# adamfilli/happy-simulator

Hardware: AMD Instinct MI355X
Metric: committed events/sec (whole node), 65 536-server M/M/1 grid (higher is better)
Workload: dtype int64+f64

## Files before the change

### happy_simulator_amd/csrc/hs_device.hpp

```cpp
#pragma once

#include <hip/hip_runtime.h>
#include <stdint.h>

namespace hs {

constexpr int64_t kInfNs = INT64_MAX;
constexpr double kMaxReachNs = 9.0e18;
constexpr double kLongestExpDraw = 36.8;
inline bool reach_fits_int64(int64_t horizon_ns, double step_s) { return (double)horizon_ns + step_s * 1e9 < kMaxReachNs; }

enum StreamKind : uint32_t { kStreamArrival = 0, kStreamService = 1, kStreamLink = 2, kStreamRoute = 3, kStreamKey = 4, kStreamLoss = 5 };

struct U4 { uint32_t x, y, z, w; };

__device__ __forceinline__ U4 philox4x32_10(uint32_t c0, uint32_t c1, uint32_t c2, uint32_t c3, uint32_t k0,
                                            uint32_t k1) {
#pragma unroll
    for (int r = 0; r < 10; ++r) {
        const uint64_t p0 = (uint64_t)0xD2511F53u * (uint64_t)c0, p1 = (uint64_t)0xCD9E8D57u * (uint64_t)c2;
        const uint32_t hi0 = (uint32_t)(p0 >> 32), lo0 = (uint32_t)p0;
        const uint32_t hi1 = (uint32_t)(p1 >> 32), lo1 = (uint32_t)p1;
        c0 = hi1 ^ c1 ^ k0;
        c1 = lo1;
// ... 53 lines not shown
    return __fma_rn(r1, 1e-9, q1);
}
__device__ __forceinline__ double ns_from_seconds_d(double x) { return __builtin_trunc(__dmul_rn(x, 1e9)); }
__device__ __forceinline__ double seconds_from_ns_d(double ns) {
    const double q0 = __dmul_rn(ns, 1e-9);
    const double r0 = __fma_rn(-1e9, q0, ns);
    const double q1 = __fma_rn(r0, 1e-9, q0);
    const double r1 = __fma_rn(-1e9, q1, ns);
    return __fma_rn(r1, 1e-9, q1);
}
__device__ __forceinline__ int64_t i64_from_whole_d(double d) {
    return (int64_t)((uint64_t)__double_as_longlong(__dadd_rn(d, 4503599627370496.0)) & 0xFFFFFFFFFFFFFull);
}
__device__ __forceinline__ double seconds_from_ns_ieee(int64_t ns) { return __ddiv_rn(__ll2double_rn(ns), 1e9); }

struct ConstDiv {
    double b, y;
    bool fast;
    __device__ __forceinline__ void init(double divisor) {
        b = divisor;
        y = __ddiv_rn(1.0, divisor);
        const uint64_t bits = (uint64_t)__double_as_longlong(divisor);
        const uint32_t ex = (uint32_t)(bits >> 52) & 0x7ffu;
        const bool all_ones = (bits & 0x000fffffffffffffull) == 0x000fffffffffffffull;
        fast = !all_ones && ex > 1023u - 200u && ex < 1023u + 200u && (bits >> 63) == 0;
    }
    __device__ __forceinline__ double div(double a) const {
        if (!fast) return __ddiv_rn(a, b);
        const double q0 = __dmul_rn(a, y);
        const double r0 = __fma_rn(-b, q0, a);
        const double q1 = __fma_rn(r0, y, q0);
        const double r1 = __fma_rn(-b, q1, a);
        return __fma_rn(r1, y, q1);
    }
};

struct Stream {
    uint32_t key0, key1, sid0, sid1;
    uint64_t k;
    uint32_t c2, c3;

    __device__ __forceinline__ void init(uint64_t seed, uint64_t sid, uint64_t k0) {
        key0 = (uint32_t)seed; key1 = (uint32_t)(seed >> 32);
// ... 85 lines not shown
```

### happy_simulator_amd/csrc/hs_engine.hip

```cpp
#include <hip/hip_runtime.h>

#include <cmath>
#include <cstdio>
#include <cstdlib>
#include <cstring>
#include <algorithm>
#include <new>
#include <string>
#include <vector>
#include <map>
#include <mutex>
#include <utility>

#define HS_KERNELS_MAIN
#include "hs_kernels.hpp"
#include "hs_tables_api.hpp"
#include "hs_host.hpp"
#include "hs_plan.hpp"

struct hs_engine {
    bool pending_async = false;

    hs_config cfg{};
    int C = 1;
// ... 1634 lines not shown
    if (!h || !o) return fail(h, HS_E_INVALID, "hs_engine_get_lp_stats: null argument");
    if (!h->have_stations) return fail(h, HS_E_STATE, "stations not set");
    if (h) { const int rcf = results_final(h); if (rcf) return rcf; }
    HS_HIP(h, hipSetDevice(h->cfg.device));
    HS_HIP(h, hipStreamSynchronize(h->stream));
    const size_t n = (size_t)h->cfg.n_lp;
#define DL(dst, src, T) if (o->dst) HS_HIP(h, hipMemcpy(o->dst, h->X.src, n * sizeof(T), hipMemcpyDeviceToHost))
    DL(generated, generated, int64_t); DL(accepted, accepted, int64_t); DL(dropped, dropped, int64_t);
    DL(completed, completed, int64_t); DL(rejected, rejected, int64_t); DL(total_service_s, total_service, double);
    DL(sink_received, received, int64_t); DL(queue_depth, buf, int64_t); DL(active, active, int32_t);
    DL(events, events, int64_t); DL(final_time_ns, last_time, int64_t);
#undef DL
    return HS_OK;
}

int64_t hs_engine_read_sink(hs_engine *h, int32_t lp, int64_t *t_ns, int64_t *created_ns, int64_t cap) {
    if (!h || !h->have_stations) return fail(h, HS_E_STATE, "stations not set");
    if (lp < 0 || lp >= h->cfg.n_lp) return fail(h, HS_E_INVALID, "LP index %d out of range", lp);
    if (h) { const int rcf = results_final(h); if (rcf) return rcf; }
    if (hipSetDevice(h->cfg.device) != hipSuccess || hipStreamSynchronize(h->stream) != hipSuccess)
        return fail(h, HS_E_HIP, "device synchronisation failed");
    int64_t cnt = 0;
    if (hipMemcpy(&cnt, h->X.received + lp, 8, hipMemcpyDeviceToHost) != hipSuccess) return fail(h, HS_E_HIP, "memcpy");
    if (cnt > h->L.cap) cnt = h->L.cap;
    if (cnt > cap) cnt = cap;
    if (cnt > 0) {
        int64_t *tmp = nullptr;
        if (hipMalloc(&tmp, (size_t)cnt * 8) != hipSuccess) return fail(h, HS_E_HIP, "hipMalloc of the read-back staging buffer failed");
        const int64_t *cols[2] = {h->L.sink_t, h->L.sink_created};
        int64_t *dsts[2] = {t_ns, created_ns};
        for (int c = 0; c < 2; ++c) {
            if (!dsts[c]) continue;
            hipLaunchKernelGGL(hs_gather_one, dim3((unsigned)((cnt + 255) / 256)), dim3(256), 0, h->stream, cols[c], tmp,
                               h->cfg.n_lp, lp, cnt, h->L.lp_major ? h->L.cap : (int64_t)0);
            if (hipStreamSynchronize(h->stream) != hipSuccess ||
                hipMemcpy(dsts[c], tmp, (size_t)cnt * 8, hipMemcpyDeviceToHost) != hipSuccess) {
                hipFree(tmp);
                return fail(h, HS_E_HIP, "sink read-back failed");
            }
        }
        hipFree(tmp);
    }
    return cnt;
}

int64_t hs_engine_read_sinks(hs_engine *h, int64_t *counts, int64_t *t_ns, int64_t *created_ns, int64_t cap_total) {
    if (!h || !h->have_stations) return fail(h, HS_E_STATE, "stations not set");
    if (!counts) return fail(h, HS_E_INVALID, "counts is required");
    if (h) { const int rcf = results_final(h); if (rcf) return rcf; }
    if (hipSetDevice(h->cfg.device) != hipSuccess || hipStreamSynchronize(h->stream) != hipSuccess)
        return fail(h, HS_E_HIP, "device synchronisation failed");
    const size_t n = (size_t)h->cfg.n_lp;
    if (hipMemcpy(counts, h->X.received, n * 8, hipMemcpyDeviceToHost) != hipSuccess) return fail(h, HS_E_HIP, "memcpy");
    const int64_t cap = h->L.cap;
    std::vector<int64_t> off(n);
    int64_t total = 0, maxc = 0;
// ... 11 lines not shown
        return fail(h, HS_E_HIP, "hipMalloc of the read-back staging buffers failed");
    }
    bool ok = hipMemcpy(d_off, off.data(), n * 8, hipMemcpyHostToDevice) == hipSuccess;
    const int64_t *cols[2] = {h->L.sink_t, h->L.sink_created};
    int64_t *dsts[2] = {t_ns, created_ns};
    for (int c = 0; c < 2 && ok; ++c) {
        if (!dsts[c]) continue;
        const dim3 grid((unsigned)((n + 63) / 64), (unsigned)((maxc + 63) / 64));
        hipLaunchKernelGGL(hs_gather_logs, grid, dim3(256), 0, h->stream, cols[c], h->X.received, d_off, d_out, (int)n, cap, (int)h->L.lp_major);
        ok = hipStreamSynchronize(h->stream) == hipSuccess &&
             hipMemcpy(dsts[c], d_out, (size_t)total * 8, hipMemcpyDeviceToHost) == hipSuccess;
    }
    hipFree(d_off);
    hipFree(d_out);
    if (!ok) return fail(h, HS_E_HIP, "sink read-back failed");
    return total;
}

int64_t hs_engine_read_probe(hs_engine *h, int32_t lp, int64_t *t_ns, int64_t *values, int64_t cap) {
    return hs_engine_read_probe_slot(h, lp, 0, t_ns, values, cap);
}

int hs_engine_read_source_generated(hs_engine *h, int32_t slot, int64_t *out) {
    if (!h || !h->have_stations || !out) return fail(h, HS_E_STATE, "stations not set");
    if (slot < 0 || slot > kMaxXSrc) return fail(h, HS_E_INVALID, "source slot %d out of range", slot);
    const size_t n = (size_t)h->cfg.n_lp;
    if (h) { const int rcf = results_final(h); if (rcf) return rcf; }
    HS_HIP(h, hipSetDevice(h->cfg.device));
    HS_HIP(h, hipStreamSynchronize(h->stream));
    if (slot == 0) { HS_HIP(h, hipMemcpy(out, h->X.generated, n * 8, hipMemcpyDeviceToHost)); return HS_OK; }
// ... 167 lines not shown
```

### happy_simulator_amd/csrc/hs_kernels.hpp

```cpp
#pragma once

#include <hip/hip_runtime.h>

#include "../../include/hs_engine.h"
#include "hs_netstation.hpp"
#ifdef HS_KERNELS_MAIN
#include "hs_exact.hpp"
#endif

using namespace hs;

namespace {

template <typename T>
__device__ __forceinline__ T wave_sum(T v) {
#pragma unroll
    for (int o = 32; o > 0; o >>= 1) v += __shfl_xor(v, o, 64);
    return v;
}

__device__ __forceinline__ long long shfl_xor_ll(long long v, int o) {
    int lo = (int)(unsigned)(v & 0xffffffffll), hi = (int)(v >> 32);
    lo = __shfl_xor(lo, o, 64);
    hi = __shfl_xor(hi, o, 64);
// ... 430 lines not shown
    const int lp = blockIdx.x * kBlock + tid;
    const bool live = lp < n && !producer;
    if (threadIdx.x < 12) red[threadIdx.x] = 0;
    if (threadIdx.x == 0) { red_time = INT64_MIN; red_flags[0] = 0; red_flags[1] = 0; }
    if constexpr (PC) {
        if (!producer) { pc_prod[tid] = 0; pc_cons[tid] = 0; if ((tid & 63) == 0) pc_done[tid >> 6] = 0; }
    }
    const long long cur = tot->cur_time;
    __syncthreads();

    Station<C, PF, UNI> S;
    Candidate mine;
    mine = cand_none(lp);
    if constexpr (PC) {
        if (producer) {
            const int w = tid >> 6;
            bool wants_a = false, wants_s = false;
            uint64_t gen_a = 0, gen_s = 0;
            uint32_t prod_a = 0, prod_s = 0;
            int slot_a = 0, slot_s = 0;
            if (lp < n) {
                S.tid = tid;
                S.rate = P.src_rate[lp];
                S.svc_lambda = __ddiv_rn(1.0, P.svc_mean[lp]);
                S.prof_kind = kProfConstant;
                S.init_streams(P.seed[lp], P.stream_base[lp], X.arr_k[lp], X.svc_k[lp], ring_a, ring_s);
                wants_a = P.src_kind[lp] == 1 && X.A[lp] != kInfNs;
                wants_s = P.svc_kind[lp] == 0;
                gen_a = S.arr_k; gen_s = S.svc_k;
            }
            for (;;) {
                if (__hip_atomic_load(&pc_done[w], __ATOMIC_RELAXED, __HIP_MEMORY_SCOPE_WORKGROUP)) break;
                const uint32_t c = __hip_atomic_load(&pc_cons[tid], __ATOMIC_RELAXED, __HIP_MEMORY_SCOPE_WORKGROUP);
                const uint32_t out_a = (prod_a - (c & 0xffffu)) & 0xffffu, out_s = (prod_s - (c >> 16)) & 0xffffu;
                const bool do_a = wants_a && out_a + (uint32_t)kRefill <= (uint32_t)kRing;
                const bool do_s = wants_s && out_s + (uint32_t)kRefill <= (uint32_t)kRing;
                if (!__any(do_a || do_s)) { __builtin_amdgcn_s_sleep(HS_PC_SLEEP_P); continue; }
                if (__any(do_a)) {
                    if (do_a) {
                        const uint64_t b0 = gen_a >> 1;
                        const bool odd = (gen_a & 1) != 0;
#pragma unroll
                        for (int i = 0; i < kRefill / 2; ++i) {
                            const uint64_t b = b0 + (uint64_t)i;
                            const U4 o = philox4x32_10((uint32_t)b, (uint32_t)(b >> 32), S.asid0, S.asid1, S.key0, S.key1);
                            const double v0 = S.arr_value(res53(o.x, o.y)), v1 = S.arr_value(res53(o.z, o.w));
                            if (!(i == 0 && odd)) { ring_a[slot_a][tid] = v0; slot_a = slot_a + 1 == kRing ? 0 : slot_a + 1; ++prod_a; ++gen_a; }
                            ring_a[slot_a][tid] = v1; slot_a = slot_a + 1 == kRing ? 0 : slot_a + 1; ++prod_a; ++gen_a;
                        }
                    }
                }
                if (__any(do_s)) {
                    if (do_s) {
                        const uint64_t b0 = gen_s >> 1;
                        const bool odd = (gen_s & 1) != 0;
#pragma unroll
                        for (int i = 0; i < kRefill / 2; ++i) {
                            const uint64_t b = b0 + (uint64_t)i;
                            const U4 o = philox4x32_10((uint32_t)b, (uint32_t)(b >> 32), S.ssid0, S.ssid1, S.key0, S.key1);
                            const double v0 = S.svc_value(res53(o.x, o.y)), v1 = S.svc_value(res53(o.z, o.w));
                            if (!(i == 0 && odd)) { ring_s[slot_s][tid] = v0; slot_s = slot_s + 1 == kRing ? 0 : slot_s + 1; ++prod_s; ++gen_s; }
                            ring_s[slot_s][tid] = v1; slot_s = slot_s + 1 == kRing ? 0 : slot_s + 1; ++prod_s; ++gen_s;
                        }
                    }
                }
                __hip_atomic_store(&pc_prod[tid], (prod_a & 0xffffu) | (prod_s << 16), __ATOMIC_RELEASE, __HIP_MEMORY_SCOPE_WORKGROUP);
            }
        }
    }
    if (live) {
        load_station<C, PF, UNI>(S, P, X, L, lp, n, qmem, ring_a, ring_s, tid);
        S.force_general = (flags & 1) != 0 || (PF && S.trk && (S.n_up > 0 || S.egress == kEgressServer));
    }
    const bool ended = (mode == HS_MODE_REPLICAS) ? (live && S.last_time > end_ns) : (cur > end_ns);
    bool other_pass = false;
    if constexpr (PF) {
        const int pass1 = (flags >> 28) & 7;
        if (pass1 != 0 && live && P.tabs != nullptr && P.tabs->tandem != nullptr) other_pass = P.tabs->tandem[(size_t)kMaxUp * n + lp] != pass1 - 1;
// ... 6 lines not shown
        S.last_time = S.grp_time;
        pre_group = true;
    }
    if constexpr (C == 1) {
        bool bail_reload = false;
        if (!producer) {
            const bool elig = live && !frozen && !pre_group && S.qn == 0 && S.req_eligible();
            typename Station<C, PF, UNI>::ReqCursor rc;
            rc.bail = false; rc.done = true;
            if (elig) S.req_begin(rc, end_ns);
#ifdef HS_CYCLES
            unsigned long long cyc_top = 0, cyc_step = 0, n_it = 0;
#endif
            uint32_t seen = 0;
            const uint64_t ak0 = S.arr_k, sk0 = S.svc_k;
            for (;;) {
                const bool act = elig && !rc.bail && !rc.done;
                if (!__any(act)) break;
#ifdef HS_CYCLES
                const unsigned long long c0 = __builtin_readcyclecounter();
#endif
                if constexpr (PC) {
                    const bool need_a = act && S.src_kind == 1 && S.A != kInfNs, need_s = act && S.svc_kind == 0;
                    const uint32_t ca = (uint32_t)(S.arr_k - ak0) & 0xffffu, cs = (uint32_t)(S.svc_k - sk0) & 0xffffu;
                    unsigned spins = 0;
                    while (__any((need_a && (seen & 0xffffu) == ca) || (need_s && (seen >> 16) == cs))) {
                        seen = __hip_atomic_load(&pc_prod[tid], __ATOMIC_ACQUIRE, __HIP_MEMORY_SCOPE_WORKGROUP);
                        if (__any((need_a && (seen & 0xffffu) == ca) || (need_s && (seen >> 16) == cs))) __builtin_amdgcn_s_sleep(HS_PC_SLEEP_C);
                        if (++spins > (1u << 22)) {
                            if (elig) { S.qoverflow = 1; rc.done = true; }
                            break;
                        }
                    }
                    if (spins > (1u << 22)) continue;
                } else {
                    S.top_up(act);
                }
#ifdef HS_CYCLES
                const unsigned long long c1 = __builtin_readcyclecounter();
#endif
                S.req_step(rc, act);
                if constexpr (PC) {
                    __hip_atomic_store(&pc_cons[tid], ((uint32_t)(S.arr_k - ak0) & 0xffffu) | ((uint32_t)(S.svc_k - sk0) << 16),
                                       __ATOMIC_RELAXED, __HIP_MEMORY_SCOPE_WORKGROUP);
                    seen = __hip_atomic_load(&pc_prod[tid], __ATOMIC_ACQUIRE, __HIP_MEMORY_SCOPE_WORKGROUP);
                }
#ifdef HS_CYCLES
                const unsigned long long c2 = __builtin_readcyclecounter();
                cyc_top += c1 - c0; cyc_step += c2 - c1; ++n_it;
#endif
            }
#ifdef HS_CYCLES
            if ((tid & 63) == 0) {
                atomicAdd(&tot->dbg[0], cyc_top); atomicAdd(&tot->dbg[1], cyc_step);
                atomicAdd(&tot->dbg[2], n_it); atomicAdd(&tot->dbg[3], 1ull);
            }
#endif
            if constexpr (PC) {
                if ((tid & 63) == 0) __hip_atomic_store(&pc_done[tid >> 6], 1, __ATOMIC_RELAXED, __HIP_MEMORY_SCOPE_WORKGROUP);
            }
            if (elig && !rc.bail) { S.req_finish(rc); event_order = false; }
            bail_reload = elig && rc.bail;
        }
        if constexpr (PC) __syncthreads();
        if (!producer) {
            if constexpr (PC) {
                S.ra.head = 0; S.ra.n = 0; S.rs.head = 0; S.rs.n = 0;
            }
            if (bail_reload) {
                load_station<C, PF, UNI>(S, P, X, L, lp, n, qmem, ring_a, ring_s, tid);
                S.force_general = (flags & 1) != 0 || (PF && S.trk && (S.n_up > 0 || S.egress == kEgressServer));
            }
        }
        if (!producer) {
            for (;;) {
// ... 1290 lines not shown
```

### happy_simulator_amd/csrc/hs_kernels_wave.hpp

```cpp
#pragma once

constexpr int kWaveR = 128;
constexpr int kWaveRowPad = kWaveR + 2;

namespace {

__device__ __forceinline__ double wave_shr1(double v) {
    const long long b = __double_as_longlong(v);
    int lo = (int)(unsigned)(b & 0xffffffffll), hi = (int)(b >> 32);
    lo = __builtin_amdgcn_update_dpp(lo, lo, 0x138, 0xf, 0xf, false);
    hi = __builtin_amdgcn_update_dpp(hi, hi, 0x138, 0xf, 0xf, false);
    return __longlong_as_double(((long long)hi << 32) | (unsigned)lo);
}
__device__ __forceinline__ MaxPlus mp_after(const MaxPlus &f2, const MaxPlus &f1) {
    return MaxPlus{__builtin_fmax(f2.p, f1.p + f2.q), f1.q + f2.q};
}
template <int CTRL, int RM>
__device__ __forceinline__ MaxPlus mp_scan_step(const MaxPlus &F) {
    return mp_after(F, MaxPlus{dpp_orneg<CTRL, RM>(F.p), dpp_or0<CTRL, RM>(F.q)});
}
__device__ __forceinline__ double rl64(double v, int l) {
    const long long b = __double_as_longlong(v);
    const unsigned lo = (unsigned)__builtin_amdgcn_readlane((int)(unsigned)(b & 0xffffffffll), l);
    const unsigned hi = (unsigned)__builtin_amdgcn_readlane((int)(b >> 32), l);
// ... 52 lines not shown
    for (int k = 0; k < 8; ++k) ev[k] = 0;
    uint32_t c_tick = 0, c_start = 0, c_dep = 0, seq = I.seq, seqA = I.seqA, seqD = I.seqD;
    int64_t acc2 = accepted, st2 = started, A_next_i = A, crtA2 = crtA0, rcA = I.rcA, rcD = I.rcD;
    int32_t dpA = I.dpA, dpD = I.dpD;
    if (count) {
        c_tick = O.n_tick; c_start = O.n_start; c_dep = O.n_dep;
        const uint32_t c_notify = O.n_notify, c_poll = O.n_poll;
        ev[0] = c_tick; ev[1] = c_tick; ev[2] = c_notify; ev[3] = c_poll + c_dep; ev[4] = c_start; ev[5] = c_start; ev[6] = c_dep; ev[7] = c_dep;
        acc2 = accepted + c_tick; st2 = started + c_start;
        A_next_i = A != kInfNs ? to_i64(A_next) : A;
        crtA2 = c_tick ? to_i64(a_last) : crtA0;
        if ((c_tick | c_start) != 0u) {
            const bool d_first = pend && pendS < crtA2;
            seqA = seq + (d_first ? 1u : 0u); seqD = seq + (d_first ? 0u : 1u); seq += 2u;
        }
        if (c_tick) { dpA = 1; rcA = acc2 >= 2 ? (c_tick >= 2 ? to_i64(a_last2) : L.adm[(size_t)(acc2 - 2) * n + lp]) : crtA0; }
        if (pend && pend_new) {
            const int64_t m = st2 - 1;
            if (pendS == to_i64(pendA_d)) {
                dpD = 6;
                rcD = m >= 1 ? (pend_i >= 1 ? to_i64(pendAp_d) : (m - 1 < L.cap ? L.adm[(size_t)(m - 1) * n + lp] : 0)) : crtA0;
            } else {
                dpD = 4; rcD = to_i64(pendSp_d);
            }
        }
        const int64_t Dn = pend ? pendD : kInfNs;
        const int64_t tmin = A_next_i < Dn ? A_next_i : Dn;
        if (tmin != kInfNs) {
            const bool tick_first = A_next_i < Dn || (A_next_i == Dn && (int32_t)(seqA - seqD) < 0);
            mine.t = tmin; mine.valid = 1;
            if (tick_first) { mine.t_created = crtA2; mine.depth = dpA; mine.rcrt = rcA; mine.pad = 2; }
            else { mine.t_created = pend ? pendS : 0; mine.depth = dpD; mine.rcrt = rcD; mine.pad = 0; }
            mine.rank = cand_rank(P, lp, n, mine.pad);
        }
    }
    if constexpr (FRESH) {
// ... 440 lines not shown
```

### happy_simulator_amd/csrc/hs_kernels_wide.hpp

```cpp
#pragma once

namespace {

struct MaxPlus { double p, q; };
__device__ __forceinline__ MaxPlus mp_compose(const MaxPlus &f2, const MaxPlus &f1) {
    const double a = f1.p + f2.q;
    return MaxPlus{f2.p > a ? f2.p : a, f1.q + f2.q};
}
__device__ __forceinline__ double shfl_f64(double v, int src) {
    const long long b = __double_as_longlong(v);
    int lo = (int)(unsigned)(b & 0xffffffffll), hi = (int)(b >> 32);
    lo = __shfl(lo, src, 64);
    hi = __shfl(hi, src, 64);
    return __longlong_as_double(((long long)hi << 32) | (unsigned)lo);
}
__device__ __forceinline__ int64_t shfl_i64(int64_t v, int src) {
    int lo = (int)(unsigned)(v & 0xffffffffll), hi = (int)(v >> 32);
    lo = __shfl(lo, src, 64);
    hi = __shfl(hi, src, 64);
    return ((int64_t)hi << 32) | (unsigned)lo;
}

}

// ... 306 lines not shown
        X.total_service[lp] = total_service;
        const int64_t A_next_i = run && A != kInfNs ? (int64_t)A_next : A;
        X.A[lp] = A_next_i; X.arr_time[lp] = A_next_i; X.arr_k[lp] = ak0 + (uint64_t)n_arr_total; X.svc_k[lp] = sk0 + (uint64_t)c_start;
        const int64_t crtA2 = c_tick ? (int64_t)a_last : crtA0;
        X.crtA[lp] = crtA2;
        uint32_t seq = X.seq[lp];
        uint32_t seqA = X.seqA[lp], seqD = X.seqD[lp];
        if ((c_tick | c_start) != 0u) {
            const bool d_first = pend && pendS < crtA2;
            seqA = seq + (d_first ? 1u : 0u); seqD = seq + (d_first ? 0u : 1u); seq += 2u;
            X.seqA[lp] = seqA; X.seqD[lp] = seqD; X.seq[lp] = seq;
        }
        X.last_time[lp] = lt;
        int32_t dpA = X.dpA[lp], dpD = X.dpD[lp];
        int64_t rcA = X.rcA[lp], rcD = X.rcD[lp];
        if (c_tick) { dpA = 1; rcA = acc2 >= 2 ? (c_tick >= 2 ? (int64_t)a_last2 : L.adm[(size_t)(acc2 - 2) * n + lp]) : crtA0; X.dpA[lp] = (uint8_t)dpA; X.rcA[lp] = rcA; }
        if (pend && pn) {
            const int64_t m = st2 - 1;
            const int64_t a_m = m < L.cap ? L.adm[(size_t)m * n + lp] : 0;
            if (pendS == a_m) { dpD = 6; rcD = m >= 1 ? L.adm[(size_t)(m - 1) * n + lp] : crtA0; }
            else {
                Stream st;
                st.init(((uint64_t)key1 << 32) | key0, ((uint64_t)ssid1 << 32) | ssid0, (uint64_t)(m - 1));
                const double s_prev = seconds_from_ns(ns_from_seconds(div_lambda.div(exp1_from_uniform(st.next_uniform()))));
                dpD = 4; rcD = pendS - ns_from_seconds(s_prev);
            }
            X.dpD[lp] = (uint8_t)dpD; X.rcD[lp] = rcD;
        }
        uint32_t tot_ev = 0;
#pragma unroll
        for (int k = 0; k < 8; ++k) { X.ev_kind[(size_t)k * n + lp] += ev[k]; tot_ev += ev[k]; }
        X.events[lp] += tot_ev;
        const int64_t Dn = pend ? pendD : kInfNs;
        const int64_t tmin = A_next_i < Dn ? A_next_i : Dn;
        if (tmin != kInfNs) {
// ... 148 lines not shown
```

### happy_simulator_amd/csrc/hs_plan.hpp

```cpp
#pragma once

#include <algorithm>
#include <cmath>
#include <cstdarg>
#include <cstdio>
#include <string>
#include <utility>
#include <vector>

#include "../../include/hs_engine.h"
#include "hs_netstation.hpp"
#include "hs_exact.hpp"
#include "hs_tables.hpp"

namespace hs {

inline int fail(std::string &err, int code, const char *fmt, ...) {
    char buf[512];
    va_list ap;
    va_start(ap, fmt);
    vsnprintf(buf, sizeof buf, fmt, ap);
    va_end(ap);
    err = buf;
    return code;
// ... 80 lines not shown
            if (st->src_more_stop_after_ns) p.xsrc_stop[o] = st->src_more_stop_after_ns[o];
            ++p.n_xsrc_total;
        }
    p.any_xsrc = p.n_xsrc_total > 0;
    p.uni_stations = true;
    for (int i = 0; i < n; ++i) {
        if (c.src_kind[i] != HS_SRC_POISSON || c.conc[i] != 1 || c.svc_kind[i] != HS_LAT_EXPONENTIAL || c.qcap[i] >= 0 ||
            c.src_stop[i] >= 0) { p.uni_stations = false; break; }
    }
    p.uni_grid = p.uni_stations;
    for (int i = 0; i < n && p.uni_grid; ++i) if (c.egress[i] != HS_EGRESS_SINK) p.uni_grid = false;
    p.f64_times = cfg.start_ns >= 0 && cfg.horizon_ns < (1ll << 51);
    for (int i = 0; i < n && p.f64_times; ++i)
        if (!(c.svc_mean[i] < 1e4) || !(c.src_rate[i] > 1e-3)) p.f64_times = false;
    if (!p.f64_times) p.uni_grid = false;
    if (p.any_xsrc) p.any_profile = true;
    for (int i = 0; i < n; ++i) {
        const int sk = c.src_kind[i];
        if (sk < 0 || sk > 2) return fail(err, HS_E_INVALID, "LP %d: unknown source kind %d", i, sk);
        if (sk != HS_SRC_NONE) {
            if (!st->src_rate) return fail(err, HS_E_INVALID, "src_rate is required when sources exist");
            const double r = st->src_rate[i];
            if (!(r > 0.0) || !std::isfinite(r))
                return fail(err, HS_E_INVALID, "LP %d: source rate must be > 0 (got %g)", i, r);
            if (r > 1e8) return fail(err, HS_E_UNSUPPORTED, "LP %d: source rate %g above 1e8/s is not supported", i, r);
            const double m = (r + p.xsum[(size_t)i]) * p.horizon_s;
            if (m > p.max_mean_records) p.max_mean_records = m;
            p.reach_s = std::max(p.reach_s, kLongestExpDraw / r);
        }
        const int cc = c.conc[i];
// ... 633 lines not shown
```

### happy_simulator_amd/csrc/hs_station.hpp

```cpp
#pragma once

#include "hs_device.hpp"
#include "hs_tables.hpp"

namespace hs {

enum : uint32_t { Q_PSAMPLE = 0, Q_ENQ = 1, Q_NOTIFY = 2, Q_POLL = 3, Q_DELIVER = 4, Q_TICK = 5, Q_CONT = 6, Q_SINK = 7 };
constexpr int kMaxProbes = 4;
constexpr int kRootProbe = 100;
constexpr int kMaxXSrc = 3;
constexpr int kRootXSrc = 120;
__device__ __forceinline__ uint64_t xsrc_stream_id(uint64_t lp_stream_base, int j) {
    return stream_id((1ull << 40) | (lp_stream_base << 2) | (uint64_t)j, kStreamArrival);
}
constexpr int kRootSched = 98;
constexpr int kRootInj = 200;
constexpr int kMaxUp = 4;
constexpr int kMaxInjRun = 32;
constexpr uint32_t kEgressServer = 4;

constexpr int kBlock = 256;
constexpr int kQCap = 48;
#ifndef HS_KRING
#define HS_KRING 24
// ... 99 lines not shown
    int64_t *XA, *crtX, *x_arr, *x_n;
    uint32_t *seqX;
    uint64_t *x_k;
};

struct RecordLogs {
    int64_t *adm;
    int64_t *sink_t;
    int64_t *sink_created;
    int64_t *sink_created_own;
    int64_t cap;
    int64_t *probe_t, *probe_v;
    int64_t pcap;
    int32_t lp_major;
};
__device__ __forceinline__ size_t log_at(const RecordLogs &L, int64_t k, int lp, int n) {
    return L.lp_major ? (size_t)lp * (size_t)L.cap + (size_t)k : (size_t)k * (size_t)n + (size_t)lp;
}

struct Totals {
    unsigned long long ev[15];
    unsigned long long completed;
    unsigned long long received;
    long long final_time;
    long long cur_time;
    int overflow;
    int qoverflow;
    unsigned int done;
    int undecided;
    unsigned long long dbg[4];
// ... 133 lines not shown
    static __device__ __forceinline__ int32_t rk_place(int64_t w) { return (int32_t)(w & 0xff) - (int32_t)((w >> 40) & 0xff); }
    __device__ __forceinline__ int32_t dp_next(int steps) const { return cd + steps > 255 ? 255 : cd + steps; }

    __device__ __forceinline__ void init_streams(uint64_t seed, uint64_t base, uint64_t ak, uint64_t sk,
                                                 double (*ring_a)[kBlock], double (*ring_s)[kBlock]) {
        key0 = (uint32_t)seed; key1 = (uint32_t)(seed >> 32);
        const uint64_t sa = stream_id(base, kStreamArrival), ss = stream_id(base, kStreamService);
        asid0 = (uint32_t)sa; asid1 = (uint32_t)(sa >> 32);
        ssid0 = (uint32_t)ss; ssid1 = (uint32_t)(ss >> 32);
        arr_k = ak; svc_k = sk;
        ra.reset(ring_a, tid); rs.reset(ring_s, tid);
        div_rate.init(rate);
        div_lambda.init(svc_lambda);
        inc_const = __ddiv_rn(1.0, rate);
    }
    __device__ __forceinline__ double arr_value(double u) const { return div_rate.div(exp1_from_uniform(u)); }
    __device__ __forceinline__ double svc_value(double u) const {
        const double sample = div_lambda.div(exp1_from_uniform(u));
        if constexpr (UNI) return seconds_from_ns_d(ns_from_seconds_d(sample));
        return seconds_from_ns(ns_from_seconds(sample));
    }
    template <int BLOCKS>
    __device__ __forceinline__ void refill_arr() {
        const uint64_t kg = arr_k + (uint64_t)ra.n;
        const uint64_t b0 = kg >> 1;
        const bool odd = (kg & 1) != 0;
#pragma unroll
        for (int i = 0; i < BLOCKS; ++i) {
            const uint64_t b = b0 + (uint64_t)i;
            const U4 o = philox4x32_10((uint32_t)b, (uint32_t)(b >> 32), asid0, asid1, key0, key1);
            const double v0 = arr_value(res53(o.x, o.y)), v1 = arr_value(res53(o.z, o.w));
            if (!(i == 0 && odd)) ra.push(v0);
            ra.push(v1);
// ... 75 lines not shown
        accepted++;
        buf++;
        return was_empty;
    }
    __device__ __forceinline__ bool do_notify() { ev[2]++; return active < conc; }
    __device__ __forceinline__ bool do_poll() {
        ev[3]++;
        if (buf == 0) return false;
        buf--;
        return true;
    }
    __device__ __forceinline__ uint32_t do_deliver_work(int64_t t) {
        ev[4]++;
        ev[5]++;
        const int64_t k = started++;
        if (active >= conc) { rejected++; return 0; }
        active++;
        double s; int64_t dur;
        sample_service(s, dur);
        int j = 0;
#pragma unroll
        for (int i = C - 1; i >= 0; --i) if (D[i] == kInfNs) j = i;
        const int64_t d = t + dur;
        uint32_t same = 0;
#pragma unroll
        for (int i = 0; i < C; ++i) if (i == j) {
            svc_s[i] = s;
            if (C > 1) crt[i] = (k < cap) ? adm[k * ls] : 0;
            if (d == t) { D[i] = kInfNs - 1; same = (uint32_t)i + 1; }
            else { D[i] = d; seqD[i] = seq++; crtD[i] = t; dpD[i] = dp_next(2); rcD[i] = cr; if constexpr (PF) { wkD[i] = wk + 1; lsrcD[i] = lsrc; } }
        }
// ... 497 lines not shown
        last_time = fast ? t : last_time;
        if (slow) run_group(t);
    }

    struct ReqCursor {
        int64_t T;
        int64_t Sprev, Dprev;
        int64_t nb;
        int64_t pendD, pendS;
        double pend_s;
        int64_t lt;
        uint32_t n_tick, n_notify, n_poll, n_start, n_dep;
        bool pend, blocked, bail, done;
        int64_t crtA0;
        double arr_d;
        int64_t pTa, pTd;
        uint32_t ma, md, mf;
        int64_t p_prev;
    };
    __device__ __forceinline__ bool req_eligible() const {
        return C == 1 && !force_general && qn == 0 && conc == 1 && qcap < 0 && stop_ns < 0 && svc_kind != 2 &&
               !(PF && (prof_kind != kProfConstant || n_probes > 1 || has_sched() || has_xsrc() || n_up > 0)) &&
               (egress == 0 || egress == 1) && !(buf > 0 && active == 0) && active <= 1;
    }
    __device__ __forceinline__ int64_t req_probe_time(uint32_t m) {
        return tick_lookup(tab_p[0], tab_cap, p_arr[0] + (int64_t)m, overflow);
    }
    __device__ __forceinline__ void req_probe_begin(ReqCursor &c) {
        c.ma = c.md = c.mf = 0;
        c.pTa = c.pTd = n_probes == 1 ? PA[0] : kInfNs;
// ... 38 lines not shown
                    case kProbeDropped: v = dropped; break;
                    case kProbeCompleted: v = cn; break;
                    case kProbeReceived: v = egress == 1 ? received + c_rel : received; break;
                    case kProbeGenerated: v = generated + g_rel; break;
                    default: break;
                }
                probe_t[o] = req_probe_time(c.mf);
                probe_v[o] = v;
            }
            ++c.mf;
        }
    }
    __device__ __forceinline__ void req_count_departure(ReqCursor &c, bool p, int64_t d, double s) {
        total_service = p ? __dadd_rn(total_service, s) : total_service;
        if (p && HSG(egress == 1, true)) {
            const int64_t w = sink_w + (int64_t)c.n_dep;
            if (w < cap) sink_t[w * ls] = d; else overflow = 1;
        }
        c.n_dep += p ? 1u : 0u;
        c.lt = (p && d > c.lt) ? d : c.lt;
    }
    __device__ __forceinline__ void req_begin(ReqCursor &c, int64_t T) {
        c.T = T; c.nb = buf; c.lt = last_time; c.crtA0 = crtA; c.arr_d = (double)arr_time;
        c.n_tick = c.n_notify = c.n_poll = c.n_start = c.n_dep = 0;
        c.blocked = c.bail = c.done = false;
        const bool busy = active > 0;
        c.Sprev = busy ? crtD[0] : INT64_MIN;
        c.Dprev = busy ? D[0] : INT64_MIN;
        const bool dep0 = busy && D[0] <= T;
        req_count_departure(c, dep0, D[0], svc_s[0]);
        c.pend = busy && !dep0;
        c.pendD = D[0]; c.pendS = crtD[0]; c.pend_s = svc_s[0];
        if constexpr (PF) {
            req_probe_begin(c);
            if (n_probes == 1 && busy) {
                req_probe_departures(c, true, D[0], 0);
                c.bail = c.bail || c.pTd == D[0];
            }
        }
    }
    __device__ __forceinline__ void req_step(ReqCursor &c, bool act) {
        const int64_t T = c.T;
        const bool bk = c.nb > 0 && !c.blocked;
        const bool arr = !bk && A <= T;
        const bool fin = !bk && !arr;
        const double inc = HSG(src_kind == 1, true) ? ra.peek() : inc_const;
        const double a2d = UNI ? ns_from_seconds_d(__dadd_rn(seconds_from_ns_d(c.arr_d), inc)) : 0.0;
        const int64_t a2 = UNI ? i64_from_whole_d(a2d) : ns_from_seconds(__dadd_rn(seconds_from_ns(arr_time), inc));
        const bool tie_a = arr && (A == c.Sprev || A == c.Dprev || a2 <= A);
        const bool notify = arr && c.Sprev < A;
        const bool idle = arr && c.Dprev < A;
        const int64_t Sk = bk ? c.Dprev : (A > c.Dprev ? A : c.Dprev);
        const bool st = (bk || arr) && Sk <= T;
        const double s_new = HSG(svc_kind == 0, true) ? rs.peek() : svc_const_s;
        const int64_t dur = UNI ? i64_from_whole_d(ns_from_seconds_d(s_new)) : (HSG(svc_kind == 0, true) ? ns_from_seconds(s_new) : svc_const_ns);
        const int64_t Dk = Sk + dur;
        const bool dp = st && Dk <= T;
        bool tie_p = false;
        if constexpr (PF) {
            const bool pon = act && n_probes == 1;
            if (__any(pon)) {
                req_probe_arrivals(c, pon && (arr || fin), arr ? A : T + 1, (int64_t)c.n_tick);
                req_probe_departures(c, pon && (st || fin), st ? Dk : T + 1, (int64_t)c.n_dep);
                tie_p = pon && ((arr && c.pTa == A) || (st && c.pTd == Dk));
            }
        }
        const bool bail = act && (tie_a || tie_p || (st && dur == 0));
        const bool go = act && !bail && !fin;
        c.bail = c.bail || bail;
        c.done = c.done || (act && fin);
        const bool arr_g = go && arr, st_g = go && st, dp_g = go && dp;
        if (arr_g) {
            const int64_t w = accepted + (int64_t)c.n_tick;
            if (w < cap) adm[w * ls] = A; else overflow = 1;
        }
        c.n_tick += arr_g ? 1u : 0u;
        c.n_notify += (go && notify) ? 1u : 0u;
        c.n_poll += (go && idle) ? 1u : 0u;
        c.lt = (arr_g && A > c.lt) ? A : c.lt;
        crtA = arr_g ? A : crtA;
        arr_time = arr_g ? a2 : arr_time;
        if constexpr (UNI) c.arr_d = arr_g ? a2d : c.arr_d;
        const bool pop_a = arr_g && HSG(src_kind == 1, true);
        ra.advance_if(pop_a);
        arr_k += pop_a ? 1u : 0u;
        c.n_start += st_g ? 1u : 0u;
        c.lt = (st_g && Sk > c.lt) ? Sk : c.lt;
        const bool pop_s = st_g && HSG(svc_kind == 0, true);
        rs.advance_if(pop_s);
        svc_k += pop_s ? 1u : 0u;
// ... 46 lines not shown
                if (n_probes == 1) {
                    const int64_t tP = crtP[0];
                    const bool p_before_a = tP < crtA, p_before_d = !c.pend || tP < c.pendS;
                    sP = (p_before_a ? 0u : 1u) + ((c.pend && !p_before_d) ? 1u : 0u);
                    sA += p_before_a ? 1u : 0u;
                    sD += p_before_d ? 1u : 0u;
                    seqP[0] = seq + sP;
                }
            }
            seqA = seq + sA;
            seqD[0] = seq + sD;
            seq += 3u;
        }
        if (c.n_tick != 0u) {
            dpA = 1;
            rcA = accepted >= 2 ? adm[(accepted - 2) * ls] : c.crtA0;
        }
        if (c.pend && c.n_start != 0u) {
            const int64_t m = started - 1;
            const int64_t a_m = m < cap ? adm[m * ls] : 0;
            if (c.pendS == a_m) {
                dpD[0] = 6;
                rcD[0] = m >= 1 ? adm[(m - 1) * ls] : c.crtA0;
            } else {
                double s_prev = svc_const_s;
                if (HSG(svc_kind == 0, true)) {
                    Stream st;
                    st.init(((uint64_t)key1 << 32) | key0, ((uint64_t)ssid1 << 32) | ssid0, (uint64_t)(m - 1));
                    s_prev = svc_value(st.next_uniform());
                }
                dpD[0] = 4;
                rcD[0] = c.pendS - ns_from_seconds(s_prev);
            }
        }
        last_time = c.lt > last_probe ? c.lt : last_probe;
    }
};

// ... 3 lines not shown
```

Before: 605.8 billion.

## Add wave-uniform interior fast path for M/M/1 steps and block-aligned Philox refills

Adds an interior fast path to the request stepping loop. When every active lane's next event is a plain arrival, start and departure inside the window, the lanes take a streamlined step that skips the tie, probe and blocking logic, and the counters are folded in at the end. The producer refill now works in whole Philox blocks aligned to the refill size, removing per-element odd and wrap checks. It also uses the unchecked fast division when the uniform grid is selected, and keeps running log pointers instead of recomputing indices. Separately, rejected admissions are now marked in the admission log and filtered on host read-back, a correctness and feature change that adds a little branching.

```diff
diff --git a/happy_simulator_amd/csrc/hs_device.hpp b/happy_simulator_amd/csrc/hs_device.hpp
--- a/happy_simulator_amd/csrc/hs_device.hpp
+++ b/happy_simulator_amd/csrc/hs_device.hpp
@@ -91,19 +91,25 @@
 }
 __device__ __forceinline__ double seconds_from_ns_ieee(int64_t ns) { return __ddiv_rn(__ll2double_rn(ns), 1e9); }
 
+__host__ __device__ inline bool const_div_fast(double divisor) {
+    const uint64_t bits = __builtin_bit_cast(uint64_t, divisor);
+    const uint32_t ex = (uint32_t)(bits >> 52) & 0x7ffu;
+    const bool all_ones = (bits & 0x000fffffffffffffull) == 0x000fffffffffffffull;
+    return !all_ones && ex > 1023u - 200u && ex < 1023u + 200u && (bits >> 63) == 0;
+}
 struct ConstDiv {
     double b, y;
     bool fast;
     __device__ __forceinline__ void init(double divisor) {
         b = divisor;
         y = __ddiv_rn(1.0, divisor);
-        const uint64_t bits = (uint64_t)__double_as_longlong(divisor);
-        const uint32_t ex = (uint32_t)(bits >> 52) & 0x7ffu;
-        const bool all_ones = (bits & 0x000fffffffffffffull) == 0x000fffffffffffffull;
-        fast = !all_ones && ex > 1023u - 200u && ex < 1023u + 200u && (bits >> 63) == 0;
+        fast = const_div_fast(divisor);
     }
     __device__ __forceinline__ double div(double a) const {
         if (!fast) return __ddiv_rn(a, b);
+        return div_fast(a);
+    }
+    __device__ __forceinline__ double div_fast(double a) const {
         const double q0 = __dmul_rn(a, y);
         const double r0 = __fma_rn(-b, q0, a);
         const double q1 = __fma_rn(r0, y, q0);
diff --git a/happy_simulator_amd/csrc/hs_engine.hip b/happy_simulator_amd/csrc/hs_engine.hip
--- a/happy_simulator_amd/csrc/hs_engine.hip
+++ b/happy_simulator_amd/csrc/hs_engine.hip
@@ -1672,6 +1672,24 @@
     return HS_OK;
 }
 
+static int skip_rejected_admissions(hs_engine *h, int32_t lp, int64_t cnt, int64_t rej, int64_t *created) {
+    int64_t want = cnt + rej;
+    if (want > h->L.cap) want = h->L.cap;
+    int64_t *tmp = nullptr;
+    if (hipMalloc(&tmp, (size_t)want * 8) != hipSuccess) return fail(h, HS_E_HIP, "hipMalloc of the read-back staging buffer failed");
+    std::vector<int64_t> all((size_t)want);
+    hipLaunchKernelGGL(hs_gather_one, dim3((unsigned)((want + 255) / 256)), dim3(256), 0, h->stream, h->L.adm, tmp, h->cfg.n_lp, lp, want,
+                       h->L.lp_major ? h->L.cap : (int64_t)0);
+    const bool ok = hipStreamSynchronize(h->stream) == hipSuccess &&
+                    hipMemcpy(all.data(), tmp, (size_t)want * 8, hipMemcpyDeviceToHost) == hipSuccess;
+    hipFree(tmp);
+    if (!ok) return fail(h, HS_E_HIP, "sink read-back failed");
+    int64_t m = 0;
+    for (int64_t k = 0; k < want && m < cnt; ++k) if (all[(size_t)k] >= 0) created[m++] = all[(size_t)k];
+    return HS_OK;
+}
+static bool created_is_the_admission_log(const hs_engine *h) { return h->L.sink_created == h->L.adm; }
+
 int64_t hs_engine_read_sink(hs_engine *h, int32_t lp, int64_t *t_ns, int64_t *created_ns, int64_t cap) {
     if (!h || !h->have_stations) return fail(h, HS_E_STATE, "stations not set");
     if (lp < 0 || lp >= h->cfg.n_lp) return fail(h, HS_E_INVALID, "LP index %d out of range", lp);
@@ -1698,6 +1716,11 @@
             }
         }
         hipFree(tmp);
+        if (created_ns && created_is_the_admission_log(h)) {
+            int64_t rej = 0;
+            if (hipMemcpy(&rej, h->X.rejected + lp, 8, hipMemcpyDeviceToHost) != hipSuccess) return fail(h, HS_E_HIP, "memcpy");
+            if (rej > 0) { const int rc = skip_rejected_admissions(h, lp, cnt, rej, created_ns); if (rc) return rc; }
+        }
     }
     return cnt;
 }
@@ -1739,6 +1762,16 @@
     hipFree(d_off);
     hipFree(d_out);
     if (!ok) return fail(h, HS_E_HIP, "sink read-back failed");
+    if (created_ns && created_is_the_admission_log(h)) {
+        std::vector<int64_t> rej(n);
+        if (hipMemcpy(rej.data(), h->X.rejected, n * 8, hipMemcpyDeviceToHost) != hipSuccess) return fail(h, HS_E_HIP, "memcpy");
+        for (size_t i = 0; i < n; ++i) {
+            const int64_t c = counts[i] > cap ? cap : counts[i];
+            if (rej[i] <= 0 || c <= 0) continue;
+            const int rc = skip_rejected_admissions(h, (int32_t)i, c, rej[i], created_ns + off[i]);
+            if (rc) return rc;
+        }
+    }
     return total;
 }
 
diff --git a/happy_simulator_amd/csrc/hs_kernels.hpp b/happy_simulator_amd/csrc/hs_kernels.hpp
--- a/happy_simulator_amd/csrc/hs_kernels.hpp
+++ b/happy_simulator_amd/csrc/hs_kernels.hpp
@@ -468,8 +468,11 @@
     mine = cand_none(lp);
     if constexpr (PC) {
         if (producer) {
+            static_assert(kRing % kRefill == 0 && kRefill % 2 == 0,
+                          "HS_KRING must be a multiple of HS_KREFILL and HS_KREFILL even: a refill is whole Philox blocks that do not wrap");
             const int w = tid >> 6;
             bool wants_a = false, wants_s = false;
+            bool first_a = true, first_s = true;
             uint64_t gen_a = 0, gen_s = 0;
             uint32_t prod_a = 0, prod_s = 0;
             int slot_a = 0, slot_s = 0;
@@ -481,41 +484,45 @@
                 S.init_streams(P.seed[lp], P.stream_base[lp], X.arr_k[lp], X.svc_k[lp], ring_a, ring_s);
                 wants_a = P.src_kind[lp] == 1 && X.A[lp] != kInfNs;
                 wants_s = P.svc_kind[lp] == 0;
-                gen_a = S.arr_k; gen_s = S.svc_k;
+                const uint32_t back_a = wants_a ? (uint32_t)(S.arr_k % (uint64_t)kRefill) : 0u;
+                const uint32_t back_s = wants_s ? (uint32_t)(S.svc_k % (uint64_t)kRefill) : 0u;
+                gen_a = S.arr_k - back_a; gen_s = S.svc_k - back_s;
+                prod_a = 0u - back_a; prod_s = 0u - back_s;
+                slot_a = (int)(gen_a % (uint64_t)kRing); slot_s = (int)(gen_s % (uint64_t)kRing);
             }
             for (;;) {
                 if (__hip_atomic_load(&pc_done[w], __ATOMIC_RELAXED, __HIP_MEMORY_SCOPE_WORKGROUP)) break;
                 const uint32_t c = __hip_atomic_load(&pc_cons[tid], __ATOMIC_RELAXED, __HIP_MEMORY_SCOPE_WORKGROUP);
                 const uint32_t out_a = (prod_a - (c & 0xffffu)) & 0xffffu, out_s = (prod_s - (c >> 16)) & 0xffffu;
-                const bool do_a = wants_a && out_a + (uint32_t)kRefill <= (uint32_t)kRing;
-                const bool do_s = wants_s && out_s + (uint32_t)kRefill <= (uint32_t)kRing;
+                const bool do_a = wants_a && (first_a || out_a + (uint32_t)kRefill <= (uint32_t)kRing);
+                const bool do_s = wants_s && (first_s || out_s + (uint32_t)kRefill <= (uint32_t)kRing);
                 if (!__any(do_a || do_s)) { __builtin_amdgcn_s_sleep(HS_PC_SLEEP_P); continue; }
                 if (__any(do_a)) {
                     if (do_a) {
                         const uint64_t b0 = gen_a >> 1;
-                        const bool odd = (gen_a & 1) != 0;
 #pragma unroll
                         for (int i = 0; i < kRefill / 2; ++i) {
                             const uint64_t b = b0 + (uint64_t)i;
                             const U4 o = philox4x32_10((uint32_t)b, (uint32_t)(b >> 32), S.asid0, S.asid1, S.key0, S.key1);
-                            const double v0 = S.arr_value(res53(o.x, o.y)), v1 = S.arr_value(res53(o.z, o.w));
-                            if (!(i == 0 && odd)) { ring_a[slot_a][tid] = v0; slot_a = slot_a + 1 == kRing ? 0 : slot_a + 1; ++prod_a; ++gen_a; }
-                            ring_a[slot_a][tid] = v1; slot_a = slot_a + 1 == kRing ? 0 : slot_a + 1; ++prod_a; ++gen_a;
+                            ring_a[slot_a + 2 * i][tid] = S.arr_value(res53(o.x, o.y));
+                            ring_a[slot_a + 2 * i + 1][tid] = S.arr_value(res53(o.z, o.w));
                         }
+                        slot_a = slot_a + kRefill == kRing ? 0 : slot_a + kRefill;
+                        prod_a += (uint32_t)kRefill; gen_a += (uint64_t)kRefill; first_a = false;
                     }
                 }
                 if (__any(do_s)) {
                     if (do_s) {
                         const uint64_t b0 = gen_s >> 1;
-                        const bool odd = (gen_s & 1) != 0;
 #pragma unroll
                         for (int i = 0; i < kRefill / 2; ++i) {
                             const uint64_t b = b0 + (uint64_t)i;
                             const U4 o = philox4x32_10((uint32_t)b, (uint32_t)(b >> 32), S.ssid0, S.ssid1, S.key0, S.key1);
-                            const double v0 = S.svc_value(res53(o.x, o.y)), v1 = S.svc_value(res53(o.z, o.w));
-                            if (!(i == 0 && odd)) { ring_s[slot_s][tid] = v0; slot_s = slot_s + 1 == kRing ? 0 : slot_s + 1; ++prod_s; ++gen_s; }
-                            ring_s[slot_s][tid] = v1; slot_s = slot_s + 1 == kRing ? 0 : slot_s + 1; ++prod_s; ++gen_s;
+                            ring_s[slot_s + 2 * i][tid] = S.svc_value(res53(o.x, o.y));
+                            ring_s[slot_s + 2 * i + 1][tid] = S.svc_value(res53(o.z, o.w));
                         }
+                        slot_s = slot_s + kRefill == kRing ? 0 : slot_s + kRefill;
+                        prod_s += (uint32_t)kRefill; gen_s += (uint64_t)kRefill; first_s = false;
                     }
                 }
                 __hip_atomic_store(&pc_prod[tid], (prod_a & 0xffffu) | (prod_s << 16), __ATOMIC_RELEASE, __HIP_MEMORY_SCOPE_WORKGROUP);
@@ -552,6 +559,11 @@
 #endif
             uint32_t seen = 0;
             const uint64_t ak0 = S.arr_k, sk0 = S.svc_k;
+            if constexpr (PC) {
+                if (live) { S.ra.head = (int)(ak0 % (uint64_t)kRing); S.rs.head = (int)(sk0 % (uint64_t)kRing); }
+            }
+            uint32_t ca = 0, cs = 0;
+            uint32_t n_int = 0;
             for (;;) {
                 const bool act = elig && !rc.bail && !rc.done;
                 if (!__any(act)) break;
@@ -560,7 +572,6 @@
 #endif
                 if constexpr (PC) {
                     const bool need_a = act && S.src_kind == 1 && S.A != kInfNs, need_s = act && S.svc_kind == 0;
-                    const uint32_t ca = (uint32_t)(S.arr_k - ak0) & 0xffffu, cs = (uint32_t)(S.svc_k - sk0) & 0xffffu;
                     unsigned spins = 0;
                     while (__any((need_a && (seen & 0xffffu) == ca) || (need_s && (seen >> 16) == cs))) {
                         seen = __hip_atomic_load(&pc_prod[tid], __ATOMIC_ACQUIRE, __HIP_MEMORY_SCOPE_WORKGROUP);
@@ -577,12 +588,20 @@
 #ifdef HS_CYCLES
                 const unsigned long long c1 = __builtin_readcyclecounter();
 #endif
-                S.req_step(rc, act);
-                if constexpr (PC) {
-                    __hip_atomic_store(&pc_cons[tid], ((uint32_t)(S.arr_k - ak0) & 0xffffu) | ((uint32_t)(S.svc_k - sk0) << 16),
-                                       __ATOMIC_RELAXED, __HIP_MEMORY_SCOPE_WORKGROUP);
-                    seen = __hip_atomic_load(&pc_prod[tid], __ATOMIC_ACQUIRE, __HIP_MEMORY_SCOPE_WORKGROUP);
+                if constexpr (PC && UNI) {
+                    const auto e = S.req_eval(rc);
+                    if (!__any(act && !S.req_interior(rc, e))) {
+                        if (act) { S.req_step_interior(rc, e); ++n_int; ++ca; ++cs; }
+                    } else {
+                        S.req_step(rc, act, e);
+                        ca = (uint32_t)(S.arr_k - ak0) + n_int; cs = (uint32_t)(S.svc_k - sk0) + n_int;
+                    }
+                    ca &= 0xffffu; cs &= 0xffffu;
+                } else {
+                    S.req_step(rc, act);
+                    if constexpr (PC) { ca = (uint32_t)(S.arr_k - ak0) & 0xffffu; cs = (uint32_t)(S.svc_k - sk0) & 0xffffu; }
                 }
+                if constexpr (PC) __hip_atomic_store(&pc_cons[tid], ca | (cs << 16), __ATOMIC_RELAXED, __HIP_MEMORY_SCOPE_WORKGROUP);
 #ifdef HS_CYCLES
                 const unsigned long long c2 = __builtin_readcyclecounter();
                 cyc_top += c1 - c0; cyc_step += c2 - c1; ++n_it;
@@ -597,6 +616,7 @@
             if constexpr (PC) {
                 if ((tid & 63) == 0) __hip_atomic_store(&pc_done[tid >> 6], 1, __ATOMIC_RELAXED, __HIP_MEMORY_SCOPE_WORKGROUP);
             }
+            if constexpr (PC && UNI) S.req_fold_interior(rc, n_int);
             if (elig && !rc.bail) { S.req_finish(rc); event_order = false; }
             bail_reload = elig && rc.bail;
         }
diff --git a/happy_simulator_amd/csrc/hs_kernels_wave.hpp b/happy_simulator_amd/csrc/hs_kernels_wave.hpp
--- a/happy_simulator_amd/csrc/hs_kernels_wave.hpp
+++ b/happy_simulator_amd/csrc/hs_kernels_wave.hpp
@@ -90,12 +90,12 @@
             const bool d_first = pend && pendS < crtA2;
             seqA = seq + (d_first ? 1u : 0u); seqD = seq + (d_first ? 0u : 1u); seq += 2u;
         }
-        if (c_tick) { dpA = 1; rcA = acc2 >= 2 ? (c_tick >= 2 ? to_i64(a_last2) : L.adm[(size_t)(acc2 - 2) * n + lp]) : crtA0; }
+        if (c_tick) { dpA = 1; rcA = acc2 >= 2 ? (c_tick >= 2 ? to_i64(a_last2) : log_time(L.adm[(size_t)(acc2 - 2) * n + lp])) : crtA0; }
         if (pend && pend_new) {
             const int64_t m = st2 - 1;
             if (pendS == to_i64(pendA_d)) {
                 dpD = 6;
-                rcD = m >= 1 ? (pend_i >= 1 ? to_i64(pendAp_d) : (m - 1 < L.cap ? L.adm[(size_t)(m - 1) * n + lp] : 0)) : crtA0;
+                rcD = m >= 1 ? (pend_i >= 1 ? to_i64(pendAp_d) : (m - 1 < L.cap ? log_time(L.adm[(size_t)(m - 1) * n + lp]) : 0)) : crtA0;
             } else {
                 dpD = 4; rcD = to_i64(pendSp_d);
             }
diff --git a/happy_simulator_amd/csrc/hs_kernels_wide.hpp b/happy_simulator_amd/csrc/hs_kernels_wide.hpp
--- a/happy_simulator_amd/csrc/hs_kernels_wide.hpp
+++ b/happy_simulator_amd/csrc/hs_kernels_wide.hpp
@@ -344,11 +344,11 @@
         X.last_time[lp] = lt;
         int32_t dpA = X.dpA[lp], dpD = X.dpD[lp];
         int64_t rcA = X.rcA[lp], rcD = X.rcD[lp];
-        if (c_tick) { dpA = 1; rcA = acc2 >= 2 ? (c_tick >= 2 ? (int64_t)a_last2 : L.adm[(size_t)(acc2 - 2) * n + lp]) : crtA0; X.dpA[lp] = (uint8_t)dpA; X.rcA[lp] = rcA; }
+        if (c_tick) { dpA = 1; rcA = acc2 >= 2 ? (c_tick >= 2 ? (int64_t)a_last2 : log_time(L.adm[(size_t)(acc2 - 2) * n + lp])) : crtA0; X.dpA[lp] = (uint8_t)dpA; X.rcA[lp] = rcA; }
         if (pend && pn) {
             const int64_t m = st2 - 1;
-            const int64_t a_m = m < L.cap ? L.adm[(size_t)m * n + lp] : 0;
-            if (pendS == a_m) { dpD = 6; rcD = m >= 1 ? L.adm[(size_t)(m - 1) * n + lp] : crtA0; }
+            const int64_t a_m = m < L.cap ? log_time(L.adm[(size_t)m * n + lp]) : 0;
+            if (pendS == a_m) { dpD = 6; rcD = m >= 1 ? log_time(L.adm[(size_t)(m - 1) * n + lp]) : crtA0; }
             else {
                 Stream st;
                 st.init(((uint64_t)key1 << 32) | key0, ((uint64_t)ssid1 << 32) | ssid0, (uint64_t)(m - 1));
diff --git a/happy_simulator_amd/csrc/hs_plan.hpp b/happy_simulator_amd/csrc/hs_plan.hpp
--- a/happy_simulator_amd/csrc/hs_plan.hpp
+++ b/happy_simulator_amd/csrc/hs_plan.hpp
@@ -118,6 +118,8 @@
     for (int i = 0; i < n && p.f64_times; ++i)
         if (!(c.svc_mean[i] < 1e4) || !(c.src_rate[i] > 1e-3)) p.f64_times = false;
     if (!p.f64_times) p.uni_grid = false;
+    for (int i = 0; i < n && p.uni_grid; ++i)
+        if (!const_div_fast(c.src_rate[i]) || !const_div_fast(1.0 / c.svc_mean[i])) p.uni_grid = false;
     if (p.any_xsrc) p.any_profile = true;
     for (int i = 0; i < n; ++i) {
         const int sk = c.src_kind[i];
diff --git a/happy_simulator_amd/csrc/hs_station.hpp b/happy_simulator_amd/csrc/hs_station.hpp
--- a/happy_simulator_amd/csrc/hs_station.hpp
+++ b/happy_simulator_amd/csrc/hs_station.hpp
@@ -137,6 +137,7 @@
     int64_t pcap;
     int32_t lp_major;
 };
+__device__ __forceinline__ int64_t log_time(int64_t v) { return v < 0 ? ~v : v; }
 __device__ __forceinline__ size_t log_at(const RecordLogs &L, int64_t k, int lp, int n) {
     return L.lp_major ? (size_t)lp * (size_t)L.cap + (size_t)k : (size_t)k * (size_t)n + (size_t)lp;
 }
@@ -300,9 +301,11 @@
         div_lambda.init(svc_lambda);
         inc_const = __ddiv_rn(1.0, rate);
     }
-    __device__ __forceinline__ double arr_value(double u) const { return div_rate.div(exp1_from_uniform(u)); }
+    __device__ __forceinline__ double arr_value(double u) const {
+        return UNI ? div_rate.div_fast(exp1_from_uniform(u)) : div_rate.div(exp1_from_uniform(u));
+    }
     __device__ __forceinline__ double svc_value(double u) const {
-        const double sample = div_lambda.div(exp1_from_uniform(u));
+        const double sample = UNI ? div_lambda.div_fast(exp1_from_uniform(u)) : div_lambda.div(exp1_from_uniform(u));
         if constexpr (UNI) return seconds_from_ns_d(ns_from_seconds_d(sample));
         return seconds_from_ns(ns_from_seconds(sample));
     }
@@ -408,7 +411,11 @@
         ev[4]++;
         ev[5]++;
         const int64_t k = started++;
-        if (active >= conc) { rejected++; return 0; }
+        if (active >= conc) {
+            if (C == 1 && k < cap && adm[k * ls] >= 0) adm[k * ls] = ~adm[k * ls];
+            rejected++;
+            return 0;
+        }
         active++;
         double s; int64_t dur;
         sample_service(s, dur);
@@ -936,6 +943,8 @@
         bool pend, blocked, bail, done;
         int64_t crtA0;
         double arr_d;
+        int64_t *pa, *ps;
+        int64_t room_a, room_s;
         int64_t pTa, pTd;
         uint32_t ma, md, mf;
         int64_t p_prev;
@@ -1004,9 +1013,10 @@
     __device__ __forceinline__ void req_count_departure(ReqCursor &c, bool p, int64_t d, double s) {
         total_service = p ? __dadd_rn(total_service, s) : total_service;
         if (p && HSG(egress == 1, true)) {
-            const int64_t w = sink_w + (int64_t)c.n_dep;
-            if (w < cap) sink_t[w * ls] = d; else overflow = 1;
-        }
+            if (c.room_s > 0) *c.ps = d; else overflow = 1;
+        }
+        c.ps += p ? ls : 0;
+        c.room_s -= p ? 1 : 0;
         c.n_dep += p ? 1u : 0u;
         c.lt = (p && d > c.lt) ? d : c.lt;
     }
@@ -1014,6 +1024,8 @@
         c.T = T; c.nb = buf; c.lt = last_time; c.crtA0 = crtA; c.arr_d = (double)arr_time;
         c.n_tick = c.n_notify = c.n_poll = c.n_start = c.n_dep = 0;
         c.blocked = c.bail = c.done = false;
+        c.pa = adm + accepted * ls; c.room_a = cap - accepted;
+        c.ps = sink_t + sink_w * ls; c.room_s = cap - sink_w;
         const bool busy = active > 0;
         c.Sprev = busy ? crtD[0] : INT64_MIN;
         c.Dprev = busy ? D[0] : INT64_MIN;
@@ -1029,21 +1041,62 @@
             }
         }
     }
-    __device__ __forceinline__ void req_step(ReqCursor &c, bool act) {
+    struct ReqEval {
+        double a2d, s_new;
+        int64_t a2, dur, Sk, Dk;
+    };
+    __device__ __forceinline__ ReqEval req_eval(const ReqCursor &c) const {
+        ReqEval e;
+        const double inc = HSG(src_kind == 1, true) ? ra.peek() : inc_const;
+        e.a2d = UNI ? ns_from_seconds_d(__dadd_rn(seconds_from_ns_d(c.arr_d), inc)) : 0.0;
+        e.a2 = UNI ? i64_from_whole_d(e.a2d) : ns_from_seconds(__dadd_rn(seconds_from_ns(arr_time), inc));
+        e.s_new = HSG(svc_kind == 0, true) ? rs.peek() : svc_const_s;
+        e.dur = UNI ? i64_from_whole_d(ns_from_seconds_d(e.s_new)) : (HSG(svc_kind == 0, true) ? ns_from_seconds(e.s_new) : svc_const_ns);
+        e.Sk = A > c.Dprev ? A : c.Dprev;
+        e.Dk = (int64_t)((uint64_t)e.Sk + (uint64_t)e.dur);
+        return e;
+    }
+    __device__ __forceinline__ bool req_interior(const ReqCursor &c, const ReqEval &e) const {
+        return c.nb == 0 && e.Sk <= c.T && e.Dk <= c.T && A != c.Sprev && A != c.Dprev && e.a2 > A && e.dur != 0;
+    }
+    __device__ __forceinline__ void req_step_interior(ReqCursor &c, const ReqEval &e) {
+        static_assert(UNI && !PF, "the interior step assumes Source.poisson -> Server(Exp) -> Sink and no Probe");
+        if (c.room_a > 0) *c.pa = A; else overflow = 1;
+        c.pa += ls; c.room_a -= 1;
+        c.n_notify += c.Sprev < A ? 1u : 0u;
+        c.n_poll += c.Dprev < A ? 1u : 0u;
+        crtA = A;
+        arr_time = e.a2;
+        c.arr_d = e.a2d;
+        ra.advance_if(true);
+        rs.advance_if(true);
+        total_service = __dadd_rn(total_service, e.s_new);
+        if (c.room_s > 0) *c.ps = e.Dk; else overflow = 1;
+        c.ps += ls; c.room_s -= 1;
+        c.lt = e.Dk > c.lt ? e.Dk : c.lt;
+        c.pend = false;
+        c.Sprev = e.Sk; c.Dprev = e.Dk;
+        A = e.a2;
+    }
+    __device__ __forceinline__ void req_fold_interior(ReqCursor &c, uint32_t n_int) {
+        c.n_tick += n_int; c.n_start += n_int; c.n_dep += n_int;
+        arr_k += n_int; svc_k += n_int;
+    }
+    __device__ __forceinline__ void req_step(ReqCursor &c, bool act) { req_step(c, act, req_eval(c)); }
+    __device__ __forceinline__ void req_step(ReqCursor &c, bool act, const ReqEval &e) {
         const int64_t T = c.T;
         const bool bk = c.nb > 0 && !c.blocked;
         const bool arr = !bk && A <= T;
         const bool fin = !bk && !arr;
-        const double inc = HSG(src_kind == 1, true) ? ra.peek() : inc_const;
-        const double a2d = UNI ? ns_from_seconds_d(__dadd_rn(seconds_from_ns_d(c.arr_d), inc)) : 0.0;
-        const int64_t a2 = UNI ? i64_from_whole_d(a2d) : ns_from_seconds(__dadd_rn(seconds_from_ns(arr_time), inc));
+        const double a2d = e.a2d;
+        const int64_t a2 = e.a2;
         const bool tie_a = arr && (A == c.Sprev || A == c.Dprev || a2 <= A);
         const bool notify = arr && c.Sprev < A;
         const bool idle = arr && c.Dprev < A;
-        const int64_t Sk = bk ? c.Dprev : (A > c.Dprev ? A : c.Dprev);
+        const int64_t Sk = bk ? c.Dprev : e.Sk;
         const bool st = (bk || arr) && Sk <= T;
-        const double s_new = HSG(svc_kind == 0, true) ? rs.peek() : svc_const_s;
-        const int64_t dur = UNI ? i64_from_whole_d(ns_from_seconds_d(s_new)) : (HSG(svc_kind == 0, true) ? ns_from_seconds(s_new) : svc_const_ns);
+        const double s_new = e.s_new;
+        const int64_t dur = e.dur;
         const int64_t Dk = Sk + dur;
         const bool dp = st && Dk <= T;
         bool tie_p = false;
@@ -1061,9 +1114,10 @@
         c.done = c.done || (act && fin);
         const bool arr_g = go && arr, st_g = go && st, dp_g = go && dp;
         if (arr_g) {
-            const int64_t w = accepted + (int64_t)c.n_tick;
-            if (w < cap) adm[w * ls] = A; else overflow = 1;
-        }
+            if (c.room_a > 0) *c.pa = A; else overflow = 1;
+        }
+        c.pa += arr_g ? ls : 0;
+        c.room_a -= arr_g ? 1 : 0;
         c.n_tick += arr_g ? 1u : 0u;
         c.n_notify += (go && notify) ? 1u : 0u;
         c.n_poll += (go && idle) ? 1u : 0u;
@@ -1140,14 +1194,14 @@
         }
         if (c.n_tick != 0u) {
             dpA = 1;
-            rcA = accepted >= 2 ? adm[(accepted - 2) * ls] : c.crtA0;
+            rcA = accepted >= 2 ? (accepted - 2 < cap ? log_time(adm[(accepted - 2) * ls]) : 0) : c.crtA0;
         }
         if (c.pend && c.n_start != 0u) {
             const int64_t m = started - 1;
-            const int64_t a_m = m < cap ? adm[m * ls] : 0;
+            const int64_t a_m = m < cap ? log_time(adm[m * ls]) : 0;
             if (c.pendS == a_m) {
                 dpD[0] = 6;
-                rcD[0] = m >= 1 ? adm[(m - 1) * ls] : c.crtA0;
+                rcD[0] = m >= 1 ? log_time(adm[(m - 1) * ls]) : c.crtA0;
             } else {
                 double s_prev = svc_const_s;
                 if (HSG(svc_kind == 0, true)) {
```

New measurement: 656.4 billion (median of 6 runs). 1.08x the previous value.
